# muyangyi/SimSeg

Measured on AMD Instinct MI355X. Metric: image-text pairs/sec (train) + seg images/sec (eval), ViT-B, higher is better.
Workload: dtype fp16

## Files before the change

### simseg_amd/csrc/gemm.hip

```cpp
#include "common.h"
#include <type_traits>

namespace {

constexpr int BM = 128, BN = 128, NTHREADS = 256;
constexpr int MC_PITCH = 320;
template <int KB> struct Geo {
    static constexpr int KC_PITCH = KB + 16;
    static constexpr int NCH = KB / 16;
    static constexpr int LOADS = 128 * NCH / NTHREADS;
    static constexpr int KROWS = KB / 2;
    static constexpr int TILE_BYTES = (128 * KC_PITCH > KROWS * MC_PITCH) ? 128 * KC_PITCH : KROWS * MC_PITCH;
    static constexpr int KSTEPS = KB / 32;
};

struct GemmParams {
    const void* A; const void* B; void* C;
    int M, N, K;
    long lda, ldb, ldc;
    float alpha;
    const float* bias;
    const float* rowscale;
    const float* residual;
    long ldr;
// ... 1063 lines not shown

template <typename TO, bool TA, bool TB, int EK = 1, bool GROUPED = false, bool ATOMIC_DIRECT = false>
__global__ __launch_bounds__(512, 2) void gemm_pp_kernel(typename std::conditional<GROUPED, WgradGroupParams, GemmParams>::type arg) {
    extern __shared__ __attribute__((aligned(16))) char lds[];
    GemmParams own;
    int gkz = 0, gt = 0;
    if constexpr (GROUPED) {
        const int gq = xcd_remap(blockIdx.x, gridDim.x);
        if (gq >= arg.first[arg.n]) return;
        int i = 0;
#pragma unroll
        for (int j = 1; j < WG_MAX; ++j)
            if (j < arg.n && gq >= arg.first[j]) i = j;
        const WgradProblem& w = arg.prob[i];
        own = GemmParams{};
        own.A = w.dy; own.B = w.x; own.C = w.dw;
        own.M = w.out; own.N = w.in; own.K = arg.rows;
        own.lda = w.ld_dy; own.ldb = w.ld_x; own.ldc = w.ld_dw;
        own.alpha = 1.0f;
        own.accumulate = 1;
        own.ksplit = arg.ksplit; own.nsplit = arg.nsplit;
        own.dbg_trace = arg.dbg_trace;
        const int gtiles = (w.out >> 8) * (w.in >> 8);
        const int r = gq - arg.first[i];
        gkz = r / gtiles;
        gt = r - gkz * gtiles;
    }
    const GemmParams& p = pp_params(arg, own);
    const int tid = threadIdx.x, lane = tid & 63, wave = __builtin_amdgcn_readfirstlane(tid >> 6);
    const int grp = wave >> 2, wn = wave & 3;
    const int tiles_n = (p.N + 255) / 256;
    const int tiles = tiles_n * ((p.M + 255) / 256);
    const int q = xcd_remap(blockIdx.x, gridDim.x);
    const int kz = GROUPED ? gkz : q / tiles, t = GROUPED ? gt : q - kz * tiles;
    const int m0 = (t / tiles_n) * 256, n0 = (t % tiles_n) * 256;
    const int nk = p.K / 64;
    const int kt0 = kz * p.ksplit;
    const int ntile = min(nk, kt0 + p.ksplit) - kt0;
    const int stot = 4 * ntile;
    const char* Ab = static_cast<const char*>(p.A) + (TA ? (long)kt0 * 64 * p.lda * 2 : (long)kt0 * 128);
    const char* Bb = static_cast<const char*>(p.B) + (TB ? (long)kt0 * 64 * p.ldb * 2 : (long)kt0 * 128);
    const long astep = TA ? 64 * p.lda * 2 : 128, bstep = TB ? 64 * p.ldb * 2 : 128;
    long dA = 0, dB = 0;
    bool pf_ok = false;
    if (p.pf_next && p.nsplit == 1) {
        const int nb8 = (int)gridDim.x >> 3, rr8 = (int)gridDim.x & 7, xx = (int)blockIdx.x & 7, jj = (int)blockIdx.x >> 3;
        if (jj + 32 < nb8 + (xx < rr8 ? 1 : 0)) {
            const int tn_ = t + 32;
            const int m1 = (tn_ / tiles_n) * 256, n1 = (tn_ % tiles_n) * 256;
            if (m0 + 256 <= p.M && n0 + 256 <= p.N && m1 + 256 <= p.M && n1 + 256 <= p.N) {
                pf_ok = true;
                dA = TA ? (long)(m1 - m0) * 2 : (long)(m1 - m0) * p.lda * 2;
                dB = TB ? (long)(n1 - n0) * 2 : (long)(n1 - n0) * p.ldb * 2;
            }
        }
    }
    unsigned offA[2][2], offB[2][2];
#pragma unroll
    for (int h = 0; h < 2; ++h)
#pragma unroll
        for (int i = 0; i < 2; ++i) {
            offA[h][i] = pp_src_off<TA>(wave * 2 + i, lane, m0 + h * 128, p.M, p.lda);
            offB[h][i] = pp_src_off<TB>(wave * 2 + i, lane, n0 + h * 128, p.N, p.ldb);
            asm volatile("" : "+v"(offA[h][i]), "+v"(offB[h][i]));
        }
    const unsigned lds0 = (unsigned)(unsigned long)(__attribute__((address_space(3))) char*)lds;
    PPFrag<TA, 2> fra;
    PPFrag<TB, 1> frb;
    fra.init(0, grp * 64, lane);
    frb.init(PP_BREG, wn * 32, lane);

    f32x16 acc[4][2];
    {
        const f32x16 zero = {0.f, 0.f, 0.f, 0.f, 0.f, 0.f, 0.f, 0.f, 0.f, 0.f, 0.f, 0.f, 0.f, 0.f, 0.f, 0.f};
#pragma unroll
        for (int i = 0; i < 4; ++i)
#pragma unroll
            for (int j = 0; j < 2; ++j) acc[i][j] = zero;
    }
#define PP_STAGE(H_, KIND)                                                                                            \
    {                                                                                                                 \
        const int h_ = (H_);                                                                                          \
        const bool live_ = h_ < stot;                                                                                 \
        const int kt_ = live_ ? (h_ >> 2) : (pf_ok ? ((h_ - stot) >> 2) : ntile - 1);                                 \
        const unsigned dst_ = lds0 + (live_ ? (((KIND) & 1) ? 0 : PP_BREG) + (((h_ >> 2) & 1) * 2 + ((KIND) >> 1)) * PP_HALF : PP_DUMMY) + \
                              wave * 2048;                                                                            \
        const char* sb_ = ((KIND) & 1) ? Ab + kt_ * astep + (live_ ? 0 : dA) : Bb + kt_ * bstep + (live_ ? 0 : dB);   \
        pp_glds16(((KIND) & 1) ? offA[(KIND) >> 1][0] : offB[(KIND) >> 1][0], sb_, dst_);                             \
        pp_glds16(((KIND) & 1) ? offA[(KIND) >> 1][1] : offB[(KIND) >> 1][1], sb_, dst_ + 1024);                      \
    }
    u32x4 fa[8], fb0[4], fb1[4];
#define PP_READ_A(PAR, HALF)                                                                       \
    _Pragma("unroll") for (int i_ = 0; i_ < 2; ++i_)                                               \
        _Pragma("unroll") for (int kk_ = 0; kk_ < 4; ++kk_) fa[i_ * 4 + kk_] = fra.read(lds, ((PAR) * 2 + (HALF)) * PP_HALF, i_, kk_);
#define PP_READ_B(FB, PAR, HALF) \
    _Pragma("unroll") for (int kk_ = 0; kk_ < 4; ++kk_) FB[kk_] = frb.read(lds, ((PAR) * 2 + (HALF)) * PP_HALF, 0, kk_);
#define PP_CLUSTER(RH, CH, FB)                                                                       \
    __builtin_amdgcn_s_setprio(1);                                                                   \
    _Pragma("unroll") for (int kk_ = 0; kk_ < 4; ++kk_)                                              \
        _Pragma("unroll") for (int i_ = 0; i_ < 2; ++i_) mma<bf16_t>(acc[2 * (RH) + i_][CH], fa[i_ * 4 + kk_], FB[kk_]); \
    __builtin_amdgcn_s_setprio(0);

    if (p.stagger > 0 && blockIdx.x < 256) {
        const unsigned long long until = wall_clock64() + (unsigned long long)(((blockIdx.x >> 3) & 3) * p.stagger);
        while (wall_clock64() < until) __builtin_amdgcn_s_sleep(8);
    }
    unsigned long long tr0 = 0, tr1 = 0, tr2 = 0;
    if (p.dbg_trace) tr0 = wall_clock64();
    PP_STAGE(0, 0) PP_STAGE(1, 1) PP_STAGE(2, 2) PP_STAGE(3, 3) PP_STAGE(4, 0) PP_STAGE(5, 1) PP_STAGE(6, 2)
    wait_vm<8>();
    __builtin_amdgcn_s_barrier();
    __builtin_amdgcn_sched_barrier(0);
    if (grp == 1) __builtin_amdgcn_s_barrier();
    if (p.dbg_trace) tr1 = wall_clock64();
#define PP_BIGPHASE(READS, STAGES, RH, CA, FA_, CB, FB_)                                       \
    {                                                                                          \
    READS                                                                                  \
    STAGES                                                                                 \
    wait_vm<8>();                                                                          \
    __builtin_amdgcn_sched_barrier(0);                                                     \
    __builtin_amdgcn_s_barrier();                                                          \
    asm volatile("s_waitcnt lgkmcnt(0)" ::: "memory");                                     \
    __builtin_amdgcn_sched_barrier(0);                                                     \
    PP_CLUSTER(RH, CA, FA_)                                                                \
    PP_CLUSTER(RH, CB, FB_)                                                                \
    asm volatile("" : "+v"(acc[2 * (RH)][0]), "+v"(acc[2 * (RH) + 1][0]), "+v"(acc[2 * (RH)][1]), "+v"(acc[2 * (RH) + 1][1])); \
    __builtin_amdgcn_sched_barrier(0);                                                     \
    __builtin_amdgcn_s_barrier();                                                          \
    __builtin_amdgcn_sched_barrier(0);                                                     \
    }
    for (int tt = 0; tt < ntile; ++tt) {
        PP_BIGPHASE(PP_READ_B(fb0, 0, 0) PP_READ_A(0, 0) PP_READ_B(fb1, 0, 1), PP_STAGE(4 * tt + 7, 3), 0, 0, fb0, 1, fb1)
        frb.toggle(2 * PP_HALF);
        PP_BIGPHASE(PP_READ_A(0, 1), PP_STAGE(4 * tt + 8, 0) PP_STAGE(4 * tt + 9, 1) PP_STAGE(4 * tt + 10, 2), 1, 1, fb1, 0, fb0)
        fra.toggle(2 * PP_HALF);
    }
#undef PP_BIGPHASE
#undef PP_STAGE
#undef PP_READ_A
#undef PP_READ_B
#undef PP_CLUSTER
    if (!pf_ok) wait_vm<0>();
    if (grp == 0) __builtin_amdgcn_s_barrier();
    if (p.dbg_trace) tr2 = wall_clock64();

    const bool atomic = p.nsplit > 1;
    const bool vec_ok = epilogue_vec_ok(p, sizeof(TO));
    float* wlds = reinterpret_cast<float*>(lds) + wave * EP_WAVE_FLOATS;
    float cs[8] = {0.f, 0.f, 0.f, 0.f, 0.f, 0.f, 0.f, 0.f};
    const int c0 = n0 + wn * 32, c1 = c0 + 128;
    if constexpr (sizeof(TO) == 2) {
        const bool fastep = !atomic && vec_ok && !p.residual && !p.rowscale && p.row_group == 0 && !p.drop_thresh && !p.dbg_skip_epilogue &&
                            (p.act == 0 || p.act == 1 || (p.act == 3 && (!p.aux_blocked || (EK == 2 && p.aux_blocked == 1) || (EK == 4 && p.aux_blocked == 2))) ||
                             (((EK == 1 && !p.aux_blocked) || (EK == 3 && p.aux_blocked == 1) || (EK == 5 && p.aux_blocked == 2)) && p.act == 4 && p.aux)) && (p.act == 4 || !p.colsum) &&
                            m0 + 256 <= p.M && n0 + 256 <= p.N;
        if (fastep) {
            pp_epilogue_bf16<EK>(p, acc, reinterpret_cast<char*>(wlds), m0, c0, c1, grp, lane);
            if (pf_ok) wait_vm<16>();
            pp_trace_end(p, tid, tr0, tr1, tr2);
            return;
        }
    }
    if constexpr (sizeof(TO) == 4) {
        const bool direct = !atomic && !p.rowscale && !p.aux && p.act == 0 && p.row_group == 0 && !p.colsum && !p.accumulate &&
                            !p.dbg_skip_epilogue && m0 + 256 <= p.M && n0 + 256 <= p.N;
        if (direct) {
            pp_epilogue_f32_direct(p, acc, m0, c0, c1, grp, lane);
            if (pf_ok) wait_vm<63>();
            pp_trace_end(p, tid, tr0, tr1, tr2);
            return;
        }
    }
    if constexpr (ATOMIC_DIRECT && sizeof(TO) == 4) {
        if (atomic && !p.dbg_skip_epilogue && m0 + 256 <= p.M && n0 + 256 <= p.N) {
            pp_epilogue_atomic_direct(p, acc, m0, c0, c1, grp, lane);
            pp_trace_end(p, tid, tr0, tr1, tr2);
            return;
        }
    }
#pragma unroll 1
    for (int i = 0; i < 4; ++i) {
        f32x16 l = acc[0][0], r = acc[0][1];
#pragma unroll
        for (int ii = 1; ii < 4; ++ii)
            if (ii == i) { l = acc[ii][0]; r = acc[ii][1]; }
        if (p.dbg_trace && tid == 0) p.dbg_trace[(long)gridDim.x * 5 + (long)blockIdx.x * 4 + i] = wall_clock64();
        epilogue_block<TO>(p, l, r, wlds, m0 + (i >> 1) * 128 + grp * 64 + (i & 1) * 32, c0, c1, lane, atomic, vec_ok, cs);
    }
    flush_colsum(p, cs, c0, c1, lane);
    if (pf_ok) wait_vm<0>();
    pp_trace_end(p, tid, tr0, tr1, tr2);
}

template <typename TO, bool TA, bool TB, int EK = 1>
int launch_pp(const GemmParams& p, int splitk, hipStream_t stream) {
    constexpr int SMEM = 9 * PP_HALF;
    static bool configured = false;
    auto kern = gemm_pp_kernel<TO, TA, TB, EK>;
    if (!configured) {
        hipError_t e = hipFuncSetAttribute(reinterpret_cast<const void*>(kern), hipFuncAttributeMaxDynamicSharedMemorySize, SMEM);
        if (e != hipSuccess) return simseg_set_error("simseg_gemm: cannot reserve %d bytes of LDS: %s", SMEM, hipGetErrorString(e));
        configured = true;
    }
    const int tiles = ((p.M + 255) / 256) * ((p.N + 255) / 256);
    const int nk = p.K / 64;
    GemmParams q = p;
    if (splitk < 1) splitk = 1;
    if (splitk > nk) splitk = nk;
    q.ksplit = (nk + splitk - 1) / splitk;
    const int z = (nk + q.ksplit - 1) / q.ksplit;
    q.nsplit = z;
    hipLaunchKernelGGL(kern, dim3(tiles * z, 1, 1), dim3(512), SMEM, stream, q);
    SS_LAUNCH_CHECK("simseg_gemm(ping-pong)");
    return 0;
}

template <bool TRANS>
__device__ __forceinline__ unsigned pp2_lane_off(int piece, int lane, long ld) {
    if (!TRANS) {
        const int r = piece * 8 + (lane >> 3);
        const int c = (lane & 7) ^ kc_swz<64>(r);
        return (unsigned)((long)r * ld * 2 + c * 16);
    } else {
        const int kr = piece * 4 + (lane >> 4);
        const int c = (lane & 15) ^ ((kr & 3) << 2);
        return (unsigned)((long)kr * ld * 2 + c * 16);
    }
}

struct PP2Item { int m0, n0, ntile; const char* a0; const char* b0; };

template <bool TA, bool TB>
__device__ __forceinline__ PP2Item pp2_item(const GemmParams& p, int t, int tiles_n) {
    PP2Item it;
    it.m0 = (t / tiles_n) << 8;
    it.n0 = (t % tiles_n) << 8;
    it.ntile = p.K >> 6;
    it.a0 = static_cast<const char*>(p.A) + (TA ? (long)it.m0 * 2 : (long)it.m0 * p.lda * 2);
    it.b0 = static_cast<const char*>(p.B) + (TB ? (long)it.n0 * 2 : (long)it.n0 * p.ldb * 2);
    return it;
}

template <typename TO, bool TA, bool TB, int EK = 1>
__global__ __launch_bounds__(512, 2) void gemm_pp2_kernel(GemmParams p) {
    extern __shared__ __attribute__((aligned(16))) char lds[];
    const int tid = threadIdx.x, lane = tid & 63, wave = __builtin_amdgcn_readfirstlane(tid >> 6);
    const int grp = wave >> 2, wn = wave & 3;
    const int tiles_n = p.N >> 8;
    const int total = tiles_n * (p.M >> 8);
    const int stride = (int)gridDim.x >> 3;
    const int x = blockIdx.x & 7;
    int ord = blockIdx.x >> 3;
    const int cq = total >> 3, cr = total & 7;
    const int cnt = cq + (x < cr ? 1 : 0);
    const int base = x < cr ? x * (cq + 1) : cr * (cq + 1) + (x - cr) * cq;
    if (ord >= cnt) return;
    const long astep = TA ? 64 * p.lda * 2 : 128, bstep = TB ? 64 * p.ldb * 2 : 128;
    const long ahalf = TA ? 256 : 128 * p.lda * 2, bhalf = TB ? 256 : 128 * p.ldb * 2;
    unsigned offA[2], offB[2];
#pragma unroll
    for (int i = 0; i < 2; ++i) {
        offA[i] = pp2_lane_off<TA>(wave * 2 + i, lane, p.lda);
        offB[i] = pp2_lane_off<TB>(wave * 2 + i, lane, p.ldb);
        asm volatile("" : "+v"(offA[i]), "+v"(offB[i]));
    }
    const unsigned lds0 = (unsigned)(unsigned long)(__attribute__((address_space(3))) char*)lds;
    PPFrag<TA, 2> fra;
    PPFrag<TB, 1> frb;
    fra.init(0, grp * 64, lane);
    frb.init(PP_BREG, wn * 32, lane);

    PP2Item cur = pp2_item<TA, TB>(p, base + ord, tiles_n);
    bool has_next = ord + stride < cnt;
    PP2Item nxt = pp2_item<TA, TB>(p, base + (has_next ? ord + stride : ord), tiles_n);
    const char* sA = cur.a0;
    const char* sB = cur.b0;
    int krem = cur.ntile - 1;
    bool nxt_ok = has_next;
    unsigned spar = 0;
    bool sdummy = false;
    unsigned cpar = 0;

#define PP2_PIECE(KIND, I)                                                                                            \
    {                                                                                                                 \
        const char* sb_ = ((KIND) & 1) ? sA + ((KIND) >> 1) * ahalf : sB + ((KIND) >> 1) * bhalf;                     \
        const unsigned dst_ = lds0 + wave * 2048 + (I) * 1024 +                                                       \
                              (sdummy ? PP_DUMMY : (((KIND) & 1) ? 0 : PP_BREG) + (spar * 2 + ((KIND) >> 1)) * PP_HALF); \
        pp_glds16(((KIND) & 1) ? offA[I] : offB[I], sb_, dst_);                                                       \
    }
#define PP2_STAGE(KIND) PP2_PIECE(KIND, 0) PP2_PIECE(KIND, 1)
#define PP2_ADVANCE()                                                                    \
    {                                                                                    \
        if (krem > 0) { --krem; sA += astep; sB += bstep; }                              \
        else if (nxt_ok) { sA = nxt.a0; sB = nxt.b0; krem = nxt.ntile - 1; nxt_ok = false; } \
        else sdummy = true;                                                              \
        spar ^= 1u;                                                                      \
    }
    u32x4 fa[8], fb0[4], fb1[4];
#define PP_READ_A(HALF)                                                                            \
    _Pragma("unroll") for (int i_ = 0; i_ < 2; ++i_)                                               \
        _Pragma("unroll") for (int kk_ = 0; kk_ < 4; ++kk_) fa[i_ * 4 + kk_] = fra.read(lds, (HALF) * PP_HALF, i_, kk_);
#define PP_READ_B(FB, HALF) \
    _Pragma("unroll") for (int kk_ = 0; kk_ < 4; ++kk_) FB[kk_] = frb.read(lds, (HALF) * PP_HALF, 0, kk_);
#define PP_MMA(RH, CH, FB, KK, I) mma<bf16_t>(acc[2 * (RH) + (I)][CH], fa[(I) * 4 + (KK)], FB[KK]);
#define PP_CLUSTER(RH, CH, FB)                                                                       \
    __builtin_amdgcn_s_setprio(1);                                                                   \
    PP_MMA(RH, CH, FB, 0, 0) PP_MMA(RH, CH, FB, 0, 1)                                                \
    PP_MMA(RH, CH, FB, 1, 0) PP_MMA(RH, CH, FB, 1, 1) PP_MMA(RH, CH, FB, 2, 0)                       \
    PP_MMA(RH, CH, FB, 2, 1) PP_MMA(RH, CH, FB, 3, 0) PP_MMA(RH, CH, FB, 3, 1)                       \
     \
                                   \
    asm volatile("" : "+v"(acc[2 * (RH)][CH]), "+v"(acc[2 * (RH) + 1][CH]));                          \
    __builtin_amdgcn_s_setprio(0);
#define PP_PHASE(READS, KIND, PRE, RH, CH, FB)                                                 \
    {                                                                                          \
        READS                                                                                  \
        PRE PP2_STAGE(KIND)                                                                    \
        wait_vm<6>();                                                                          \
        __builtin_amdgcn_sched_barrier(0);                                                     \
        __builtin_amdgcn_s_barrier();                                                          \
        asm volatile("s_waitcnt lgkmcnt(0)" ::: "memory");                                     \
        __builtin_amdgcn_sched_barrier(0);                                                     \
        PP_CLUSTER(RH, CH, FB)                                                                 \
        __builtin_amdgcn_sched_barrier(0);                                                     \
        __builtin_amdgcn_s_barrier();                                                          \
        __builtin_amdgcn_sched_barrier(0);                                                     \
    }

    f32x16 acc[4][2];
    const f32x16 zero = {0.f, 0.f, 0.f, 0.f, 0.f, 0.f, 0.f, 0.f, 0.f, 0.f, 0.f, 0.f, 0.f, 0.f, 0.f, 0.f};
#pragma unroll
    for (int i = 0; i < 4; ++i)
#pragma unroll
        for (int j = 0; j < 2; ++j) acc[i][j] = zero;

    PP2_STAGE(0) PP2_STAGE(1) PP2_STAGE(2) PP2_STAGE(3)
    PP2_ADVANCE()
    PP2_STAGE(0)

    for (;;) {
        asm volatile("" : "+v"(offA[0]), "+v"(offA[1]), "+v"(offB[0]), "+v"(offB[1]));
        fra.pin(); frb.pin();
        __builtin_amdgcn_s_waitcnt(0x0F70);
        wait_vm<0>();
        __builtin_amdgcn_s_barrier();
        __builtin_amdgcn_sched_barrier(0);
        PP_READ_B(fb0, 0)
        if (grp == 1) __builtin_amdgcn_s_barrier();
        for (int tt = 0; tt < cur.ntile; ++tt) {
            PP_PHASE(PP_READ_A(0), 1, , 0, 0, fb0)
            PP_PHASE(PP_READ_B(fb1, 1), 2, , 0, 1, fb1)
            PP_PHASE(PP_READ_A(1), 3, , 1, 1, fb1)
            frb.toggle(2 * PP_HALF);
            PP_PHASE(PP_READ_B(fb1, 0), 0, PP2_ADVANCE(), 1, 0, fb0)
            fra.toggle(2 * PP_HALF);
            cpar ^= 1u;
#pragma unroll
            for (int kk = 0; kk < 4; ++kk) fb0[kk] = fb1[kk];
        }
        if (grp == 0) __builtin_amdgcn_s_barrier();
        __builtin_amdgcn_sched_barrier(0);
        const int c0 = cur.n0 + wn * 32, c1 = c0 + 128;
        if constexpr (sizeof(TO) == 2) {
            const unsigned lp = cpar ^ 1u;
            char* tl = lds + (wave < 7 ? lp * (2 * PP_HALF) + wave * 4608 : PP_BREG + (lp * 2 + 1) * PP_HALF);
            pp_epilogue_bf16<EK>(p, acc, tl, cur.m0, c0, c1, grp, lane);
        } else {
            pp_epilogue_f32_direct(p, acc, cur.m0, c0, c1, grp, lane);
        }
        if (!has_next) break;
        cur.m0 = nxt.m0; cur.n0 = nxt.n0; cur.ntile = nxt.ntile;
        ord += stride;
        has_next = ord + stride < cnt;
        nxt = pp2_item<TA, TB>(p, base + (has_next ? ord + stride : ord), tiles_n);
        nxt_ok = has_next;
#pragma unroll
        for (int i = 0; i < 4; ++i)
#pragma unroll
            for (int j = 0; j < 2; ++j) acc[i][j] = zero;
    }
    wait_vm<0>();
#undef PP_PHASE
#undef PP2_STAGE
#undef PP2_PIECE
#undef PP_MMA
#undef PP2_ADVANCE
#undef PP_READ_A
#undef PP_READ_B
#undef PP_CLUSTER
}

template <typename TO>
bool pp2_ok(const GemmParams& p, int splitk) {
    if (splitk > 1 || p.M % 256 || p.N % 256 || p.K % 64 || p.K < 128) return false;
    if (p.rowscale || p.row_group || p.dbg_skip_epilogue || p.dbg_trace) return false;
    const long tiles = (long)(p.M / 256) * (p.N / 256);
    if (tiles <= 256) return false;
    bool vec = (p.ldc % 8 == 0) && (((uintptr_t)p.C) % 16 == 0);
    if (p.bias) vec = vec && (((uintptr_t)p.bias) % 16 == 0);
    if (p.aux) vec = vec && (((uintptr_t)p.aux) % 16 == 0);
    if (p.aux_out) vec = vec && (((uintptr_t)p.aux_out) % 16 == 0);
    if (sizeof(TO) == 2)
        return vec && !p.residual && !p.drop_thresh && (p.act == 0 || p.act == 1 || p.act == 3 || (p.act == 4 && p.aux)) && (p.act == 4 || !p.colsum);
    return !p.aux && p.act == 0 && !p.colsum && !p.accumulate;
}

template <typename TO, bool TA, bool TB, int EK = 1>
int launch_pp2(const GemmParams& p, hipStream_t stream, int reserve = 0) {
    constexpr int SMEM = 9 * PP_HALF;
    static bool configured = false;
    static int blocks = 0;
    auto kern = gemm_pp2_kernel<TO, TA, TB, EK>;
    if (!configured) {
        hipError_t e = hipFuncSetAttribute(reinterpret_cast<const void*>(kern), hipFuncAttributeMaxDynamicSharedMemorySize, SMEM);
        if (e != hipSuccess) return simseg_set_error("simseg_gemm: cannot reserve %d bytes of LDS: %s", SMEM, hipGetErrorString(e));
        int dev = 0, cus = 0;
        if (hipGetDevice(&dev) != hipSuccess || hipDeviceGetAttribute(&cus, hipDeviceAttributeMultiprocessorCount, dev) != hipSuccess || cus < 8)
            return simseg_set_error("simseg_gemm: cannot read the CU count");
        blocks = cus & ~7;
        configured = true;
    }
    GemmParams q = p;
    q.ksplit = p.K / 64; q.nsplit = 1;
    const int nb = reserve > 0 ? ((blocks - reserve) & ~7) : blocks;
    hipLaunchKernelGGL(kern, dim3(nb < 8 ? 8 : nb, 1, 1), dim3(512), SMEM, stream, q);
    SS_LAUNCH_CHECK("simseg_gemm(persistent ping-pong)");
    return 0;
}



thread_local int g_gemm_variant = 0;
thread_local int g_gemm_last_variant = 0;
thread_local unsigned long long* g_gemm_debug_trace = nullptr;

template <typename T, typename TO, int WM, int WK>
__global__ __launch_bounds__(256) void gemm_small_kernel(GemmParams p) {
    constexpr int TM = 32 * WM, TN = 64, NSTAGE = 4;
    constexpr int PA = TM / 8, PB = TN / 8;
    constexpr int PPW = (PA + PB) / 4;
    constexpr int STAGE = (TM + TN) * 128;
    constexpr int KPW = 4 / WK;
    static_assert(WM * WK == 4 && (PA + PB) % 4 == 0, "four waves");
    static_assert(NSTAGE * STAGE >= (WK - 1) * WM * 8192 + WM * EP_WAVE_FLOATS * 4, "ring doubles as reduction + epilogue scratch");
    extern __shared__ __attribute__((aligned(16))) char lds[];
    const int tid = threadIdx.x, lane = tid & 63, wave = __builtin_amdgcn_readfirstlane(tid >> 6);
    const int wm = wave % WM, wk = wave / WM;
    const int tiles_n = (p.N + TN - 1) / TN;
    const int t = xcd_remap(blockIdx.x, gridDim.x);
    const int m0 = (t / tiles_n) * TM, n0 = (t % tiles_n) * TN;
    const int nk = (int)((long)p.K * (long)sizeof(T) / 128);

    const char* src[PPW];
    int dst[PPW];
#pragma unroll
    for (int i = 0; i < PPW; ++i) {
        const int pi = wave * PPW + i;
        const bool isb = pi >= PA;
        const int pr = isb ? pi - PA : pi;
        const int r = pr * 8 + (lane >> 3);
        const int c = (lane & 7) ^ ((r >> 1) & 7);
        int gr = (isb ? n0 : m0) + r;
        const int lim = isb ? p.N : p.M;
        gr = gr < lim ? gr : lim - 1;
        src[i] = static_cast<const char*>(isb ? p.B : p.A) + ((long)gr * (isb ? p.ldb : p.lda)) * (long)sizeof(T) + c * 16;
        dst[i] = (isb ? TM * 128 : 0) + pr * 1024;
    }
    auto issue = [&](int stage, int kt) {
#pragma unroll
        for (int i = 0; i < PPW; ++i)
            __builtin_amdgcn_global_load_lds((const __attribute__((address_space(1))) void*)(src[i] + (long)kt * 128),
                                             (__attribute__((address_space(3))) void*)(lds + stage * STAGE + dst[i]), 16, 0, 0);
    };
    f32x16 acc0, acc1;
#pragma unroll
    for (int r = 0; r < 16; ++r) { acc0[r] = 0.f; acc1[r] = 0.f; }
#pragma unroll
    for (int s = 0; s < NSTAGE - 1; ++s)
        if (s < nk) issue(s, s);
    int stage = 0;
    for (int kt = 0; kt < nk; ++kt) {
        const int ahead = min(NSTAGE - 2, nk - 1 - kt);
        if (ahead >= 2) wait_vm<2 * PPW>();
        else if (ahead == 1) wait_vm<PPW>();
        else wait_vm<0>();
        __builtin_amdgcn_s_barrier();
        __builtin_amdgcn_sched_barrier(0);
        if (kt + NSTAGE - 1 < nk) {
            int ns = stage + NSTAGE - 1; ns = ns >= NSTAGE ? ns - NSTAGE : ns;
            issue(ns, kt + NSTAGE - 1);
        }
        const char* sa = lds + stage * STAGE;
        const char* sb = sa + TM * 128;
#pragma unroll
        for (int kq = 0; kq < KPW; ++kq) {
            const int c = 2 * (wk * KPW + kq) + (lane >> 5);
            const int ra = wm * 32 + (lane & 31), rb = lane & 31;
            const u32x4 fa = *reinterpret_cast<const u32x4*>(sa + ra * 128 + ((c ^ ((ra >> 1) & 7)) << 4));
            const u32x4 fb0 = *reinterpret_cast<const u32x4*>(sb + rb * 128 + ((c ^ ((rb >> 1) & 7)) << 4));
            const u32x4 fb1 = *reinterpret_cast<const u32x4*>(sb + (rb + 32) * 128 + ((c ^ (((rb + 32) >> 1) & 7)) << 4));
            mma<T>(acc0, fa, fb0);
            mma<T>(acc1, fa, fb1);
        }
        stage = stage + 1 == NSTAGE ? 0 : stage + 1;
    }
    __builtin_amdgcn_s_barrier();
    if (WK > 1) {
        float* red = reinterpret_cast<float*>(lds);
        if (wk > 0) {
            float* dstp = red + ((wk - 1) * WM + wm) * 2048 + lane;
#pragma unroll
            for (int r = 0; r < 16; ++r) { dstp[r * 64] = acc0[r]; dstp[(16 + r) * 64] = acc1[r]; }
        }
        __syncthreads();
        if (wk > 0) return;
#pragma unroll
        for (int g = 0; g < WK - 1; ++g) {
            const float* sp = red + (g * WM + wm) * 2048 + lane;
#pragma unroll
            for (int r = 0; r < 16; ++r) { acc0[r] += sp[r * 64]; acc1[r] += sp[(16 + r) * 64]; }
        }
    }
    float* wlds = reinterpret_cast<float*>(lds + (WK - 1) * WM * 8192) + wm * EP_WAVE_FLOATS;
    float cs[8] = {0.f, 0.f, 0.f, 0.f, 0.f, 0.f, 0.f, 0.f};
    epilogue_block<TO>(p, acc0, acc1, wlds, m0 + wm * 32, n0, n0 + 32, lane, false, epilogue_vec_ok(p, sizeof(TO)), cs);
    flush_colsum(p, cs, n0, n0 + 32, lane);
}

template <typename T, typename TO, int WM, int WK>
int launch_small(const GemmParams& p, hipStream_t stream) {
    constexpr int SMEM = 4 * (32 * WM + 64) * 128;
    static bool configured = false;
    auto kern = gemm_small_kernel<T, TO, WM, WK>;
    if (!configured) {
        hipError_t e = hipFuncSetAttribute(reinterpret_cast<const void*>(kern), hipFuncAttributeMaxDynamicSharedMemorySize, SMEM);
        if (e != hipSuccess) return simseg_set_error("simseg_gemm: cannot reserve %d bytes of LDS: %s", SMEM, hipGetErrorString(e));
        configured = true;
    }
    GemmParams q = p;
    q.ksplit = 0; q.nsplit = 1;
    const int tiles = ((p.M + 32 * WM - 1) / (32 * WM)) * ((p.N + 63) / 64);
    hipLaunchKernelGGL(kern, dim3(tiles), dim3(256), SMEM, stream, q);
    SS_LAUNCH_CHECK("simseg_gemm(small)");
    return 0;
}

template <typename T, typename TO>
int dispatch_small(const GemmParams& p, hipStream_t s) {
    const long t64 = (long)((p.M + 63) / 64) * ((p.N + 63) / 64);
    if (t64 >= 192) return launch_small<T, TO, 2, 2>(p, s);
    return launch_small<T, TO, 1, 4>(p, s);
}

template <typename TO, bool TB, typename F>
int with_pp_kind(const GemmParams& p, F&& f) {
    if constexpr (sizeof(TO) == 2) {
        if constexpr (!TB) {
            if (p.act == 3 && p.aux_blocked == 1) return f(std::integral_constant<int, 2>{});
            if (p.act == 3 && p.aux_blocked == 2) return f(std::integral_constant<int, 4>{});
        } else {
            if (p.act == 4 && p.aux_blocked == 1) return f(std::integral_constant<int, 3>{});
            if (p.act == 4 && p.aux_blocked == 2) return f(std::integral_constant<int, 5>{});
        }
        if (!p.aux_blocked && p.act != 4) return f(std::integral_constant<int, 0>{});
    }
    if (p.aux_blocked) return simseg_set_error("simseg_gemm: act 5 / 7 is a forward (x . W^T) epilogue, act 6 / 8 a dgrad (d . W) epilogue, both with 16-bit outputs");
    return f(std::integral_constant<int, 1>{});
}

template <typename TO, bool TA, bool TB>
int dispatch_bf16(const GemmParams& p, int splitk, bool aligned, hipStream_t s) {
    const int sel = g_gemm_variant;
    const bool big_ok = aligned && p.K % 64 == 0 && p.M >= 256 && p.N >= 128;
    const int nk64 = p.K / 64;
    const int kper = (nk64 + (splitk > 1 ? splitk : 1) - 1) / (splitk > 1 ? splitk : 1);
    const int tiles256 = ((p.M + 255) / 256) * ((p.N + 255) / 256);
    if constexpr (TA && sizeof(TO) == 4) {
        if ((sel == 0 || sel == 3) && big_ok && p.accumulate && splitk > 1 && p.M % 256 == 0 && p.N % 256 == 0 && tiles256 <= 128) {
            int sk = 256 / tiles256;
            if (nk64 / sk < 16 && nk64 >= 64) sk = nk64 / 16;
            if (nk64 / sk >= 16 && tiles256 * sk >= 96) {
                g_gemm_last_variant = 3;
                return launch_pp<TO, TA, TB>(p, sk, s);
            }
        }
    }
    if constexpr (!TA) {
        const int pad_n = ((p.N + 255) / 256) * 256 - p.N;
        const bool n_fits = pad_n * 6 <= p.N || kper >= 40;
        const bool pp_auto = tiles256 >= 96 && n_fits && (kper >= 12 || (kper >= 6 && tiles256 >= 1024));
        if (big_ok && (sel == 0 ? pp_auto : ((sel == 3 || sel == 10) && p.K >= 128))) {
            static const int reserve = getenv("SIMSEG_GEMM_PP2_RESERVE") ? atoi(getenv("SIMSEG_GEMM_PP2_RESERVE")) : 0;
            if ((sel == 10 || (sel == 0 && tiles256 >= 600)) && (p.act != 4 || p.aux_blocked) && pp2_ok<TO>(p, splitk)) {
                g_gemm_last_variant = 10;
                return with_pp_kind<TO, TB>(p, [&](auto ek) {
                    return launch_pp2<TO, TA, TB, decltype(ek)::value == 1 ? 0 : decltype(ek)::value>(p, s, sel == 0 ? reserve : 0);
                });
            }
            g_gemm_last_variant = 3;
            return with_pp_kind<TO, TB>(p, [&](auto ek) { return launch_pp<TO, TA, TB, decltype(ek)::value>(p, splitk, s); });
        }
    }
    if (p.aux_blocked)
        return simseg_set_error("simseg_gemm: act 5 - 8 (tile-blocked saved derivative) need the 256x256 ping-pong kernel; this call does not dispatch to it");
    if constexpr (!TA && !TB) {
        const long t128 = (long)((p.M + 127) / 128) * ((p.N + 127) / 128);
        const bool ring_ok = aligned && p.K % 64 == 0 && p.M >= 128 && p.N >= 128 && splitk <= 1;
        if (ring_ok && (sel == 5 || (sel == 0 && t128 >= 160 && t128 <= 256))) {
            g_gemm_last_variant = 5;
            return launch_large<TO, TA, TB, 64, 4, 128, 128, 2, 2, 1>(p, splitk, s);
        }
    }
    g_gemm_last_variant = 1;
    return launch<bf16_t, TO, TA, TB>(p, splitk, s);
}

}

extern "C" int simseg_gemm_last_variant(void) {
    SS_HALF_FWD(simseg_gemm_last_variant); return g_gemm_last_variant; }

extern "C" int simseg_debug_gemm_trace(void* buf) { g_gemm_debug_trace = static_cast<unsigned long long*>(buf); return 0; }

extern "C" int simseg_set_gemm_variant(int v) {
    SS_CHECK(v == 0 || v == 1 || v == 3 || v == 4 || v == 5 || v == 10,
             "set_gemm_variant: %d is not a kernel selection (0 = auto, 1 = 128x128, 3 = ping-pong per tile, 4 = small-problem, 5 = 128x128 ring, 10 = persistent ping-pong)", v);
#ifndef SS_HALF
    simseg_set_gemm_variant_h16(v);
#endif
    g_gemm_variant = v;
    return 0;
}

extern "C" int simseg_patch_text_sim(const void* x, const void* text, float* out, int64_t M, int64_t C, int64_t K, int dtype,
                                     float eps, int normalize, void* stream) {
    SS_HALF_FWD(simseg_patch_text_sim, x, text, out, M, C, K, dtype, eps, normalize, stream);
    SS_CHECK(x && text && out, "patch_text_sim: null pointer");
    SS_CHECK(M > 0 && C > 0 && C <= 256 && K > 0 && M < (1ll << 31), "patch_text_sim: need 1 <= C <= 256 (got C=%lld)", (long long)C);
    SS_CHECK(dtype == 0 || dtype == 1, "patch_text_sim: dtype must be 0 (fp32) or 1 (bf16)");
    const int epc = dtype == 0 ? 4 : 8;
    SS_CHECK(K % epc == 0 && ((uintptr_t)x % 16) == 0 && ((uintptr_t)text % 16) == 0, "patch_text_sim: K must be a multiple of %d and the operands 16-byte aligned", epc);
    if (dtype == 0) return dispatch_simmap<float>(x, text, out, (int)M, (int)C, (int)K, eps, normalize, (hipStream_t)stream);
    return dispatch_simmap<bf16_t>(x, text, out, (int)M, (int)C, (int)K, eps, normalize, (hipStream_t)stream);
}

extern "C" int simseg_gemm_aux_blocked_ok(int64_t M, int64_t N, int64_t K) {
    if (M <= 0 || N <= 0 || K <= 0 || M % 256 || N % 256 || K % 64 || K < 768) return 0;
    return (M / 256) * (N / 256) >= 96;
}

static thread_local int g_wgrad_group_last = 0;
extern "C" int simseg_wgrad_group_last(void) {
    SS_HALF_FWD(simseg_wgrad_group_last); return g_wgrad_group_last; }

extern "C" int simseg_gemm_wgrad_group(const int64_t* problems, int n, int64_t rows, int slices, void* stream) {
    SS_HALF_FWD(simseg_gemm_wgrad_group, problems, n, rows, slices, stream);
    g_wgrad_group_last = 0;
    SS_CHECK(problems && n >= 1 && n <= WG_MAX, "simseg_gemm_wgrad_group: 1..%d problems", WG_MAX);
    SS_CHECK(rows > 0 && rows < (1ll << 31) && slices >= 1, "simseg_gemm_wgrad_group: bad rows %lld / slices %d", (long long)rows, slices);
    if (rows % 64 != 0) return 0;
    const int nk = (int)(rows / 64);
    if (nk / slices < 16) return 0;
    WgradGroupParams g;
    memset(&g, 0, sizeof(g));
    g.ksplit = (nk + slices - 1) / slices;
    g.nsplit = (nk + g.ksplit - 1) / g.ksplit;
    long blocks = 0;
    for (int i = 0; i < n; ++i) {
        const int64_t* d = problems + 8 * i;
        WgradProblem& w = g.prob[i];
        SS_CHECK(d[0] && d[1] && d[2], "simseg_gemm_wgrad_group: null operand in problem %d", i);
        const int64_t out = d[3], in = d[4];
        if (out <= 0 || in <= 0 || out % 256 || in % 256 || out >= (1ll << 31) || in >= (1ll << 31)) return 0;
        if (d[5] < out || d[6] < in || d[7] < in || d[5] % 8 || d[6] % 8 || d[7] % 4) return 0;
        if ((uintptr_t)d[0] % 16 || (uintptr_t)d[1] % 16 || (uintptr_t)d[2] % 16) return 0;
        if (64 * d[5] * 2 >= (1ll << 31) || 64 * d[6] * 2 >= (1ll << 31)) return 0;
        w.dy = (const void*)(uintptr_t)d[0]; w.x = (const void*)(uintptr_t)d[1]; w.dw = (float*)(uintptr_t)d[2];
        w.out = (int)out; w.in = (int)in; w.ld_dy = d[5]; w.ld_x = d[6]; w.ld_dw = d[7];
        g.first[i] = (int)blocks;
        blocks += (out / 256) * (in / 256) * g.nsplit;
        if (blocks >= (1l << 24)) return 0;
    }
    for (int i = n; i <= WG_MAX; ++i) g.first[i] = (int)blocks;
    g.n = n; g.rows = (int)rows;
    g.dbg_trace = g_gemm_debug_trace;
    constexpr int SMEM = 9 * PP_HALF;
    auto kern = gemm_pp_kernel<float, true, true, 1, true, true>;
    static bool configured = false;
// ... 74 lines not shown
```

Baseline: 6120.

## Merge four-phase ping-pong GEMM loop into two larger MMA phases

Restructures the ping-pong GEMM main loop from four barrier-delimited phases per K-tile into two bigger phases. Each phase now issues two MMA clusters and groups several global-to-LDS stage loads together. The vmcnt wait threshold and the prologue staging order change to match. The aim is to halve the number of workgroup barriers and waitcnt stalls per tile and give the scheduler longer MMA runs. In exchange, loads and LDS reads overlap MMAs at a coarser grain, and the new stage ordering could raise register pressure or cause hazards.

```diff
diff --git a/simseg_amd/csrc/gemm.hip b/simseg_amd/csrc/gemm.hip
--- a/simseg_amd/csrc/gemm.hip
+++ b/simseg_amd/csrc/gemm.hip
@@ -1389,26 +1389,23 @@
         _Pragma("unroll") for (int kk_ = 0; kk_ < 4; ++kk_) fa[i_ * 4 + kk_] = fra.read(lds, (HALF) * PP_HALF, i_, kk_);
 #define PP_READ_B(FB, HALF) \
     _Pragma("unroll") for (int kk_ = 0; kk_ < 4; ++kk_) FB[kk_] = frb.read(lds, (HALF) * PP_HALF, 0, kk_);
-#define PP_MMA(RH, CH, FB, KK, I) mma<bf16_t>(acc[2 * (RH) + (I)][CH], fa[(I) * 4 + (KK)], FB[KK]);
 #define PP_CLUSTER(RH, CH, FB)                                                                       \
     __builtin_amdgcn_s_setprio(1);                                                                   \
-    PP_MMA(RH, CH, FB, 0, 0) PP_MMA(RH, CH, FB, 0, 1)                                                \
-    PP_MMA(RH, CH, FB, 1, 0) PP_MMA(RH, CH, FB, 1, 1) PP_MMA(RH, CH, FB, 2, 0)                       \
-    PP_MMA(RH, CH, FB, 2, 1) PP_MMA(RH, CH, FB, 3, 0) PP_MMA(RH, CH, FB, 3, 1)                       \
-     \
-                                   \
-    asm volatile("" : "+v"(acc[2 * (RH)][CH]), "+v"(acc[2 * (RH) + 1][CH]));                          \
+    _Pragma("unroll") for (int kk_ = 0; kk_ < 4; ++kk_)                                              \
+        _Pragma("unroll") for (int i_ = 0; i_ < 2; ++i_) mma<bf16_t>(acc[2 * (RH) + i_][CH], fa[i_ * 4 + kk_], FB[kk_]); \
     __builtin_amdgcn_s_setprio(0);
-#define PP_PHASE(READS, KIND, PRE, RH, CH, FB)                                                 \
+#define PP_BIGPHASE(READS, STAGES, RH, CA, FA_, CB, FB_)                                       \
     {                                                                                          \
         READS                                                                                  \
-        PRE PP2_STAGE(KIND)                                                                    \
-        wait_vm<6>();                                                                          \
+        STAGES                                                                                 \
+        wait_vm<8>();                                                                          \
         __builtin_amdgcn_sched_barrier(0);                                                     \
         __builtin_amdgcn_s_barrier();                                                          \
         asm volatile("s_waitcnt lgkmcnt(0)" ::: "memory");                                     \
         __builtin_amdgcn_sched_barrier(0);                                                     \
-        PP_CLUSTER(RH, CH, FB)                                                                 \
+        PP_CLUSTER(RH, CA, FA_)                                                                \
+        PP_CLUSTER(RH, CB, FB_)                                                                \
+        asm volatile("" : "+v"(acc[2 * (RH)][0]), "+v"(acc[2 * (RH) + 1][0]), "+v"(acc[2 * (RH)][1]), "+v"(acc[2 * (RH) + 1][1])); \
         __builtin_amdgcn_sched_barrier(0);                                                     \
         __builtin_amdgcn_s_barrier();                                                          \
         __builtin_amdgcn_sched_barrier(0);                                                     \
@@ -1422,8 +1419,6 @@
         for (int j = 0; j < 2; ++j) acc[i][j] = zero;
 
     PP2_STAGE(0) PP2_STAGE(1) PP2_STAGE(2) PP2_STAGE(3)
-    PP2_ADVANCE()
-    PP2_STAGE(0)
 
     for (;;) {
         asm volatile("" : "+v"(offA[0]), "+v"(offA[1]), "+v"(offB[0]), "+v"(offB[1]));
@@ -1432,18 +1427,15 @@
         wait_vm<0>();
         __builtin_amdgcn_s_barrier();
         __builtin_amdgcn_sched_barrier(0);
-        PP_READ_B(fb0, 0)
+        PP2_ADVANCE()
+        PP2_STAGE(0) PP2_STAGE(1) PP2_STAGE(2)
         if (grp == 1) __builtin_amdgcn_s_barrier();
         for (int tt = 0; tt < cur.ntile; ++tt) {
-            PP_PHASE(PP_READ_A(0), 1, , 0, 0, fb0)
-            PP_PHASE(PP_READ_B(fb1, 1), 2, , 0, 1, fb1)
-            PP_PHASE(PP_READ_A(1), 3, , 1, 1, fb1)
+            PP_BIGPHASE(PP_READ_B(fb0, 0) PP_READ_A(0) PP_READ_B(fb1, 1), PP2_STAGE(3), 0, 0, fb0, 1, fb1)
             frb.toggle(2 * PP_HALF);
-            PP_PHASE(PP_READ_B(fb1, 0), 0, PP2_ADVANCE(), 1, 0, fb0)
+            PP_BIGPHASE(PP_READ_A(1), if (tt + 1 < cur.ntile) { PP2_ADVANCE() PP2_STAGE(0) PP2_STAGE(1) PP2_STAGE(2) }, 1, 1, fb1, 0, fb0)
             fra.toggle(2 * PP_HALF);
             cpar ^= 1u;
-#pragma unroll
-            for (int kk = 0; kk < 4; ++kk) fb0[kk] = fb1[kk];
         }
         if (grp == 0) __builtin_amdgcn_s_barrier();
         __builtin_amdgcn_sched_barrier(0);
@@ -1467,10 +1459,9 @@
             for (int j = 0; j < 2; ++j) acc[i][j] = zero;
     }
     wait_vm<0>();
-#undef PP_PHASE
+#undef PP_BIGPHASE
 #undef PP2_STAGE
 #undef PP2_PIECE
-#undef PP_MMA
 #undef PP2_ADVANCE
 #undef PP_READ_A
 #undef PP_READ_B
```

Measured after the change: 6165 (median of 6 runs). Within noise of the previous version (+0.7%).
